# COPT-Public/LoRADS

Measured on AMD Instinct MI355X. Metric: ADMM iters/sec (+ inner CG-iters/sec), single-block n=20000 r=40, higher is better.
Workload: dtype f64

## Files before the change

include/lorads_hip.h:

```cpp
#ifndef LORADS_HIP_H
#define LORADS_HIP_H

#include <stdint.h>

#ifdef __cplusplus
extern "C" {
#endif

typedef struct lorads_hip_ctx lorads_hip_ctx;

typedef struct {
    int32_t n;
    int32_t rank;
    int32_t nrow;
    const int32_t *row_idx;
    const int32_t *a_ptr;
    const int32_t *a_row;
    const int32_t *a_col;
    const double *a_val;
    int32_t c_nnz;
    const int32_t *c_row;
    const int32_t *c_col;
    const double *c_val;
    int32_t is_lp;
// ... 70 lines not shown

int lorads_hip_primal_topk(lorads_hip_ctx *ctx, int32_t src, int32_t blk, int32_t nq, const int32_t *row, int32_t col_lo, int32_t col_hi,
                           int32_t k, int32_t smallest, int32_t include_diag, const int64_t *skip_ptr, const int32_t *skip_col,
                           int32_t *idx, double *val, int32_t *found);

int lorads_hip_alm_to_admm(lorads_hip_ctx *ctx);
int lorads_hip_average_uv_to_v(lorads_hip_ctx *ctx);
int lorads_hip_scale_obj(lorads_hip_ctx *ctx, double s);
int lorads_hip_resize_rank(lorads_hip_ctx *ctx, const int32_t *new_rank);
int lorads_hip_set_mat(lorads_hip_ctx *ctx, int32_t which, int32_t blk, const double *colmajor);
int lorads_hip_get_mat(lorads_hip_ctx *ctx, int32_t which, int32_t blk, double *colmajor);
int lorads_hip_set_vec(lorads_hip_ctx *ctx, int32_t which, const double *v);
int lorads_hip_get_vec(lorads_hip_ctx *ctx, int32_t which, double *v);
int lorads_hip_set_allreduce(lorads_hip_ctx *ctx, lorads_hip_allreduce_fn fn, void *user);
void *lorads_hip_stream(lorads_hip_ctx *ctx);
int lorads_hip_set_allreduce_stream_ordered(lorads_hip_ctx *ctx, int32_t on);
int lorads_hip_set_separable(lorads_hip_ctx *ctx, int32_t on);
typedef int (*lorads_hip_scalar_exchange_fn)(void *user, double *vals, int32_t n);
int lorads_hip_set_scalar_exchange(lorads_hip_ctx *ctx, lorads_hip_scalar_exchange_fn fn, void *user);
int lorads_hip_selfcheck_allreduce(lorads_hip_ctx *ctx);

int lorads_hip_sync(lorads_hip_ctx *ctx);
int lorads_hip_spec_front_stats(lorads_hip_ctx *ctx, int64_t out[4]);
int lorads_hip_row_deal_stats(lorads_hip_ctx *ctx, int32_t block, int out[3]);
int lorads_hip_wt_stores(lorads_hip_ctx *ctx, int *mask);

#ifdef __cplusplus
}
#endif
#endif
```

lorads_amd/csrc/hip/kernels.inc:

```
template <int LG, bool V2, int NS>
struct Slice {
    static constexpr int W = V2 ? 2 : 1;
    __device__ static __forceinline__ void load(const double *__restrict__ row, int r, int lane, double (&v)[NS][W]) {
#pragma unroll
        for (int c = 0; c < NS; ++c) {
            const int j = (lane + c * LG) * W;
            const bool ok = j < r;
            const int jc = ok ? j : 0;
            if (V2) {
                const double2 t = *(const double2 *)(row + jc);
                v[c][0] = ok ? t.x : 0.0;
                v[c][W - 1] = ok ? t.y : 0.0;
            } else {
                const double t = row[jc];
                v[c][0] = ok ? t : 0.0;
            }
        }
    }
};

enum { WT_R0 = 1, WT_RHS = 2, WT_CONTRIB = 4, WT_CG0 = 8, WT_AVG = 16, WT_OUT = 32, WT_ALL = 63,
       WT_DEFAULT = WT_R0 | WT_RHS | WT_CG0 | WT_AVG };
__device__ __forceinline__ void store16(double *p, size_t off, double a, double b, bool wt) {
    if (wt) {
// ... 827 lines not shown
    DS rho, rho_dual;
    int dual_on;
    int wmode;
    double *contrib;
    CGState *reset;
    int nreset;
    int wt;
};
__device__ __forceinline__ void front_cw_weights(const FrontCwArgs &A, double rho, double rho_dual, int i, double a, double &c1, double &c2) {
    const int g = A.row_idx ? A.row_idx[i] : i;
    const double cs0 = A.csum[g], bb = A.b[g], lam0 = A.lambda[g], cvv = A.cv[i], wu = A.w_uv[i];
    double m1;
    if (A.wmode == W_ADMM_V) {
        const double cs = cs0 + (wu - cvv);
        m1 = ((cs - bb) - wu) * rho - lam0;
    } else {
        double lam = lam0;
        if (A.dual_on) { const double l = lam0 + rho_dual * bb; lam = l + (-rho_dual) * cs0; }
        m1 = ((cs0 - bb) - cvv) * rho - lam;
    }
    c1 = a * m1;
    c2 = a * wu;
}
template <int NS, int EW, int KC = 0>
__global__ __launch_bounds__(TPB) void k_front_cw(int n, int rpw, FrontCwArgs A, const double *__restrict__ X, int r,
                                                  const double *__restrict__ xin, double *__restrict__ out,
                                                  double *__restrict__ rhs_out, double *__restrict__ part,
                                                  double *__restrict__ part_b, Guard g, Deferred d) {
    constexpr int LG = 8, W = 2, NH = EW / 8;
    using SL = Slice<LG, true, NS>;
    __shared__ double sh[8];
    extern __shared__ __attribute__((aligned(16))) double2 slotc[];
    if (A.reset && blockIdx.x == 0 && threadIdx.x < A.nreset) A.reset[threadIdx.x].done = 0;
    const Gate gt = gate_load(g);
    const double rho = dsv(A.rho), rho_dual = A.dual_on ? dsv(A.rho_dual) : 0.0;
    DefPriv dv{};
    if (d.st) dv = deferred_private(d);
    const int grp = threadIdx.x / LG, row = blockIdx.x * rpw + grp, lane = threadIdx.x % LG, l8 = lane & 7;
    const bool act = grp < rpw && row < n;
    const int rowc = act ? row : 0;
    const size_t base = (size_t)rowc * r;
    const int c0 = A.fc_ptr[rowc], c1e = act ? A.fc_ptr[rowc + 1] : c0;
    const int a0 = A.sl_ptr[rowc], a1r = A.sl_ptr[rowc + 1];
    const int a1 = act ? a1r : a0;
    const int cnt = a1 - a0;
    const size_t eb = (size_t)rowc * EW + l8;
    int qc[NH], kc[NH], dc[NH];
    double ac[NH];
#pragma unroll
    for (int h = 0; h < NH; ++h) { qc[h] = A.ell_col[eb + 8 * h]; kc[h] = A.ell_con[eb + 8 * h]; ac[h] = A.ell_a[eb + 8 * h]; dc[h] = A.ell_dst[eb + 8 * h]; }
    int tn = c0 + l8, tc = tn < c1e ? tn : (c1e > 0 ? c1e - 1 : 0);
    int qn = A.fc_col[tc];
    double svn = A.fc_val[tc];
    double xi[NS][W], rh[NS][W];
    SL::load(X + base, r, lane, xi);
    SL::load(xin + base, r, lane, rh);
    double k1[NH], k2[NH];
#pragma unroll
    for (int h = 0; h < NH; ++h) {
        front_cw_weights(A, rho, rho_dual, kc[h], ac[h], k1[h], k2[h]);
        const bool mine = l8 + 8 * h < cnt;
// ... 112 lines not shown
#pragma unroll
                    for (int c = 0; c < NS; ++c)
#pragma unroll
                        for (int w = 0; w < W; ++w) dsum += r0[c][w] * v[u][c][w];
                    dsum = group_sum<LG>(dsum);
                    mine = l8 == u0 + u ? dsum : mine;
                }
            }
            if (live && l8 + 8 * h < cnt2) store8(A.contrib, (size_t)dc[h], ac[h] * mine, A.wt & WT_CONTRIB);
        }
    }
    for (int t = a0 + EW; t < a1b; ++t) {
        double v[NS][W], dsum = 0.0;
        SL::load(X + (size_t)A.sl_col[t] * r, r, lane, v);
#pragma unroll
        for (int c = 0; c < NS; ++c)
#pragma unroll
            for (int w = 0; w < W; ++w) dsum += r0[c][w] * v[c][w];
        dsum = group_sum<LG>(dsum);
        if (live && l8 == 0) store8(A.contrib, (size_t)A.sl_dst[t], A.sl_a[t] * dsum, A.wt & WT_CONTRIB);
    }
    double two[2] = {act ? local : 0.0, act ? local_b : 0.0};
    block_sum_n<2>(two, sh);
    if (live && threadIdx.x == 0) { part[blockIdx.x] = two[0]; part_b[blockIdx.x] = two[1]; }
}

__global__ __launch_bounds__(TPB) void k_wsum(int nrow, int cw, const double *__restrict__ contrib, double *__restrict__ w_out, Guard g,
                                              InitArgs ia, int dual_on, DS rho_dual_s, int m_all,
                                              const double *__restrict__ b, const double *__restrict__ csum,
                                              double *__restrict__ lambda, double *__restrict__ part_ww = nullptr,
                                              CGState *reset = nullptr, int nreset = 0) {
    __shared__ double sh[8];
    if (reset && blockIdx.x == 0 && threadIdx.x < nreset) reset[threadIdx.x].done = 0;
    const Gate gt = gate_load(ia.st ? Guard{nullptr, g.need} : g);
    double iv[2] = {0.0, 0.0};
    if (ia.st) init_private(ia, iv);
    const int i = (blockIdx.x * TPB + threadIdx.x) / 8, lane = threadIdx.x & 7;
    const bool act = i < nrow;
    const int ic = act ? i : 0;
    const double *cp = contrib + (size_t)ic * cw;
    double s = 0.0;
    for (int t = lane; t < cw; t += 32) {
        double v[4];
#pragma unroll
        for (int u = 0; u < 4; ++u) v[u] = cp[t + 8 * u < cw ? t + 8 * u : lane];
#pragma unroll
        for (int u = 0; u < 4; ++u) s += t + 8 * u < cw ? v[u] : 0.0;
// ... 926 lines not shown
    double acc = 0.0;
    for (int col = threadIdx.x; col < ncols; col += TPB) {
        double w = cobj[col];
        for (int t = ptr[col]; t < ptr[col + 1]; ++t) w += -lambda[grow[t]] * a[t];
        acc += fabs(w < 0.0 ? w : 0.0);
    }
    acc = block_sum(acc, sh);
    if (threadIdx.x == 0) *out = acc;
}

__global__ __launch_bounds__(TPB) void k_publish(const unsigned long long *__restrict__ src, int nwords, unsigned long long *dst,
                                                 unsigned long long *flag, unsigned long long *seq_dev) {
    const unsigned long long seq = *seq_dev + 1;
    for (int i = threadIdx.x; i < nwords; i += TPB) dst[i] = src[i];
    __threadfence_system();
    __syncthreads();
    if (threadIdx.x == 0) {
        *seq_dev = seq;
        __atomic_store_n(flag, seq, __ATOMIC_RELEASE);
        __threadfence_system();
    }
}

struct EvalFinalArgs {
    const double *part_v, *part_d, *obj_part;
    int np, nobj;
    double *out;
    Guard g;
};
__global__ __launch_bounds__(TPB) void k_publish_final(EvalFinalArgs fa, const unsigned long long *src, int nwords,
                                                       unsigned long long *dst, unsigned long long *flag, unsigned long long *seq_dev) {
    __shared__ double sh[12];
    const unsigned long long seq = *seq_dev + 1;
    constexpr int PW = 4;
    unsigned long long pre[PW];
#pragma unroll
    for (int k = 0; k < PW; ++k) {
        const int i = threadIdx.x + k * TPB;
        pre[k] = __builtin_nontemporal_load(src + (i < nwords ? i : 0));
    }
    const bool live = !blocked(fa.g);
    const double *const pp[3] = {fa.part_v, fa.part_d, fa.obj_part ? fa.obj_part : fa.part_v};
    const int nn[3] = {fa.np, fa.np, fa.obj_part ? fa.nobj : 0};
    double t3[3];
    private_partials_n<3>(pp, nn, t3);
    block_sum_n<3>(t3, sh);
    const double v = t3[0], d = t3[1], o = t3[2];
    if (live && threadIdx.x == 0) { fa.out[0] = v; fa.out[1] = d; if (fa.obj_part) fa.out[2] = o; }
    const bool own = (const double *)src == fa.out;
#pragma unroll
    for (int k = 0; k < PW; ++k) {
        const int i = threadIdx.x + k * TPB;
        if (i >= nwords) continue;
        unsigned long long w = pre[k];
        if (live && own) {
            if (i == 0) w = (unsigned long long)__double_as_longlong(v);
            else if (i == 1) w = (unsigned long long)__double_as_longlong(d);
            else if (i == 2 && fa.obj_part) w = (unsigned long long)__double_as_longlong(o);
        }
        dst[i] = w;
    }
    if (!own || nwords > PW * TPB) {
        __threadfence();
        __syncthreads();
        for (int i = threadIdx.x; i < nwords; i += TPB) dst[i] = __builtin_nontemporal_load(src + i);
    }
    __threadfence_system();
    __syncthreads();
    if (threadIdx.x == 0) {
        *seq_dev = seq;
        __atomic_store_n(flag, seq, __ATOMIC_RELEASE);
        __threadfence_system();
    }
}
struct SepExtra;
__global__ __launch_bounds__(TPB) void k_publish_sep(const double *buf, double *scal, int with_obj, int nex, double *ex0, double *ex1,
                                                     double *ex2, double *ex3, const unsigned long long *src, int nwords,
                                                     unsigned long long *dst, unsigned long long *flag, unsigned long long *seq_dev) {
    const unsigned long long seq = *seq_dev + 1;
    if (threadIdx.x == 0) {
        scal[0] = buf[0];
        scal[1] = buf[1];
        if (with_obj) scal[2] = buf[2];
        scal[5] = buf[3];
        double *const ex[4] = {ex0, ex1, ex2, ex3};
        for (int k = 0; k < nex; ++k) *ex[k] = buf[4 + k];
    }
    __threadfence();
    __syncthreads();
    for (int i = threadIdx.x; i < nwords; i += TPB) dst[i] = __builtin_nontemporal_load(src + i);
    __threadfence_system();
    __syncthreads();
    if (threadIdx.x == 0) {
        *seq_dev = seq;
        __atomic_store_n(flag, seq, __ATOMIC_RELEASE);
        __threadfence_system();
// ... 616 lines not shown
```

lorads_amd/csrc/hip/lorads_hip.hip:

```cpp
#include <hip/hip_runtime.h>

#include <fcntl.h>
#include <sys/file.h>
#include <unistd.h>

#include <algorithm>
#include <chrono>
#include <cmath>
#include <cstdint>
#include <cstdio>
#include <cstring>
#include <map>
#include <string>
#include <atomic>
#include <mutex>
#include <thread>
#include <tuple>
#include <type_traits>
#include <utility>
#include <vector>

#include "lorads_hip.h"
#include "lorads_hip_dev.h"

// ... 607 lines not shown
    bool opt_dense_cache = true;
    bool opt_front_diag = true;
    bool opt_eval_diag = true;
    bool opt_fold_avg = true;
    bool opt_tile_update = true;
    bool avg_folded = false;
    bool opt_front_lds = true;
    bool opt_front_cw = true;
    bool opt_fuse_cg0 = true;
    int opt_row_deal = -1, row_deal_cus = 0;
    int opt_wt_stores = WT_DEFAULT;
    bool opt_spec_front = true;
    struct SpecFront {
        bool live = false;
        bool dual_seen = false;
        double rho = 0.0, rho_dual = 0.0;
        int wmode = 0;
        unsigned long long epoch = 0;
        CGState *reset = nullptr;
        int nreset = 0;
    } spec;
    unsigned long long spec_epoch = 0;
    long long n_spec_enq = 0, n_spec_adopt = 0, n_spec_discard = 0, n_spec_blocked = 0;
    bool opt_exact_refresh = false, opt_split_front = false;
    bool final_pending = false;
    EvalFinalArgs final_args;
    double *scal = nullptr;
    CGState *st = nullptr;
    CGState *st_shadow = nullptr;
    bool opt_lazy_scalars = true;
    bool opt_seg_carry_init = true;
    lorads_hip_scalar_exchange_fn sx = nullptr;
    void *sx_user = nullptr;
    bool sx_pending = false;
    int sx_with_obj = 0;
    long long n_sx = 0;
    bool opt_seg_virt = true;
    bool opt_seg_carry_dual = true;
    bool opt_seg_carry_restart = true;
    double *seg_rr_alt = nullptr;
    int *seg_tile_info = nullptr;
    bool opt_seg_carry = true;
    int *seg_tile_cone = nullptr;
    CGState *h_st = nullptr;
    double *h_scal = nullptr;
    std::vector<Ring> ring;
// ... 114 lines not shown
    c->opt_gram = env_on("LORADS_LBFGS_GRAM");
    c->opt_gram_single = getenv("LORADS_LBFGS_GRAM") && getenv("LORADS_LBFGS_GRAM")[0] == '2';
    c->opt_fuse_dir = env_on("LORADS_FUSE_DIR");
    c->opt_entry_bip = env_on("LORADS_ENTRY_BIP");
    c->opt_seg_carry = env_on("LORADS_SEG_CARRY");
    c->opt_seg_carry_init = env_on("LORADS_SEG_CARRY_INIT");
    c->opt_seg_virt = env_on("LORADS_SEG_VIRT");
    c->opt_seg_carry_dual = env_on("LORADS_SEG_CARRY_DUAL");
    c->opt_seg_carry_restart = env_on("LORADS_SEG_CARRY_RESTART");
    c->opt_cw_quad = env_on("LORADS_CW_QUAD");
    c->opt_front_cw = env_on("LORADS_FRONT_CW");
    c->opt_fuse_cg0 = env_on("LORADS_FUSE_CG0");
    c->opt_front_lds = env_on("LORADS_FRONT_LDS");
    {
        const char *v = getenv("LORADS_ROW_DEAL");
        c->opt_row_deal = (!v || !v[0] || v[0] == 'a') ? -1 : std::max(0, std::min(32, atoi(v)));
        int dev = 0;
        HC(hipGetDevice(&dev));
        HC(hipDeviceGetAttribute(&c->row_deal_cus, hipDeviceAttributeMultiprocessorCount, dev));
        if (getenv("LORADS_ROW_DEAL_CUS")) c->row_deal_cus = std::max(1, atoi(getenv("LORADS_ROW_DEAL_CUS")));
    }
    if (getenv("LORADS_WT_STORES") && getenv("LORADS_WT_STORES")[0]) c->opt_wt_stores = atoi(getenv("LORADS_WT_STORES")) & WT_ALL;
    c->opt_spec_front = env_on("LORADS_SPEC_FRONT");
    if (getenv("LORADS_SPEC_WINDOW")) c->spec_window = std::max(1, std::min(8, atoi(getenv("LORADS_SPEC_WINDOW"))));
    c->opt_fold_avg = env_on("LORADS_FOLD_AVG");
    c->opt_tile_update = env_on("LORADS_TILE_UPDATE");
    c->opt_eval_diag = env_on("LORADS_EVAL_DIAG");
    c->opt_front_diag = env_on("LORADS_FRONT_DIAG");
    c->opt_dense_cache = env_on("LORADS_DENSE_CACHE");
    c->opt_fuse_eval = env_on("LORADS_FUSE_EVAL");
    c->opt_dense_rem = env_on("LORADS_DENSE_REM");
    c->opt_exact_refresh = env_set("LORADS_EXACT_REFRESH");
    c->opt_split_front = env_set("LORADS_SPLIT_FRONT");
    c->scal = (double *)c->ctrl;
    c->st = (CGState *)(c->ctrl + 64 * sizeof(double));
    c->h_scal = (double *)c->h_ctrl;
    c->h_st = (CGState *)(c->h_ctrl + 64 * sizeof(double));
    HC(hipMemset(c->lambda, 0, sizeof(double) * (size_t)std::max(c->m, 1)));
    HC(hipMemset(c->csum, 0, sizeof(double) * (size_t)(c->m + 2)));
    HC(hipMemset(c->q12, 0, sizeof(double) * (size_t)(2 * c->m + 2)));
    HC(hipMemset(c->scal, 0, sizeof(double) * 64));
    HC(hipMemset(c->ring_ab, 0, sizeof(double) * (size_t)2 * c->L));
    HC(hipMemset(c->st, 0, sizeof(CGState) * (size_t)std::max(2 * c->nb, 1)));
    if (M.alloc(&c->st_shadow, (size_t)std::max(2 * c->nb, 1))) return 1;
    HC(hipMemset(c->st_shadow, 0, sizeof(CGState) * (size_t)std::max(2 * c->nb, 1)));
    c->persist = new PersistPlan();
// ... 862 lines not shown
    for (int i = 0; i < 16; ++i) ticks[i] = 0;
    if (c->persist && c->persist->valid && c->persist->stamps && c->persist_stamps) {
        HC(hipMemcpy(c->persist->h_stamps, c->persist->stamps, sizeof(unsigned long long) * 16, hipMemcpyDeviceToHost));
        for (int i = 0; i < 16; ++i) ticks[i] = c->persist->h_stamps[i];
        HC(hipMemset(c->persist->stamps, 0, sizeof(unsigned long long) * 16));
    }
    c->persist_stamps = enable != 0;
    return 0;
}

int lorads_hip_presolve_stats(lorads_hip_ctx *c, int64_t stats[2]) {
    spec_touch(c);
    stats[0] = c->n_dev_patterns;
    stats[1] = c->n_checked_patterns;
    return 0;
}

int lorads_hip_spec_front_stats(lorads_hip_ctx *c, int64_t out[4]) {
    if (!c || !out) return fail_msg("spec_front_stats: bad argument");
    out[0] = c->n_spec_enq; out[1] = c->n_spec_adopt; out[2] = c->n_spec_discard; out[3] = c->n_spec_blocked;
    return 0;
}

int lorads_hip_row_deal_stats(lorads_hip_ctx *c, int32_t k, int out[3]) {
    if (!c || !out) return fail_msg("row_deal_stats: bad argument");
    if (k < 0 || k >= c->nb) return fail_msg("bad block");
    const RowDeal rd = row_deal_of(c, c->blk[k]);
    out[0] = rd.rpw; out[1] = rd.grid; out[2] = c->row_deal_cus;
    return 0;
}

int lorads_hip_wt_stores(lorads_hip_ctx *c, int *mask) {
    if (!c || !mask) return fail_msg("wt_stores: bad argument");
    *mask = c->opt_wt_stores;
    return 0;
}

int lorads_hip_graph_stats(lorads_hip_ctx *c, int64_t stats[4]) {
    spec_touch(c);
    stats[0] = c->graphs ? c->graphs->n_capture : 0;
    stats[1] = c->graphs ? c->graphs->n_replay : 0;
    stats[2] = c->graphs ? (int64_t)c->graphs->map.size() : 0;
    stats[3] = graph_ok(c) ? 1 : 0;
    return 0;
}

// ... 24 lines not shown
```

lorads_amd/csrc/hip/sweep.inc:

```
#define LAUNCH_LDS(kern, grid, lds, ...)                                                             \
    do {                                                                                             \
        const int grid__ = (int)(grid);                                                              \
        if (c->pend.must_flush()) c->pend.flush(c);                                                  \
        if (grid__ > 0) { ++c->n_launch; hipLaunchKernelGGL(kern, dim3(grid__), dim3(TPB), (size_t)(lds), c->stream, __VA_ARGS__); } \
    } while (0)
#define LAUNCH(kern, grid, ...) LAUNCH_LDS(kern, grid, 0, __VA_ARGS__)
#include "pending.inc"

struct Shape {
    int lg, v2, ns;
};
inline Shape shape_for(int r) {
    Shape s;
    s.v2 = use_v2(r);
    s.lg = lg_for(r);
    const int w = s.v2 ? 2 : 1;
    s.ns = (r + s.lg * w - 1) / (s.lg * w);
    return s;
}
#define NS_SWITCH(LGV, V2V, ns, ...)                                     \
    switch (ns) {                                                        \
    case 1: { constexpr int LG_ = LGV; constexpr bool V2_ = V2V; constexpr int NS_ = 1; __VA_ARGS__; } break; \
    case 2: { constexpr int LG_ = LGV; constexpr bool V2_ = V2V; constexpr int NS_ = 2; __VA_ARGS__; } break; \
    case 3: { constexpr int LG_ = LGV; constexpr bool V2_ = V2V; constexpr int NS_ = 3; __VA_ARGS__; } break; \
// ... 377 lines not shown
};

struct Solve {
    Block *B;
    double *x;
    const double *V;
    CGState *st;
    Guard front;
    size_t len;
    int gv;
    int tile = 0, tile_w = 0;
};

FrontCwArgs front_cw_args(lorads_hip_ctx *c, const Block &B, double rho, int wmode) {
    FrontCwArgs A{};
    A.fc_ptr = B.fc_ptr; A.fc_col = B.fc_col; A.fc_val = B.fc_val; A.sl_ptr = B.cadj_ptr; A.sl_col = B.cadj_col; A.sl_con = B.cadj_con;
    A.sl_a = B.cadj_a; A.ell_col = B.cell_col; A.ell_con = B.cell_con; A.ell_a = B.cell_a; A.ell_dst = B.cell_dst; A.sl_dst = B.cadj_dst; A.csum = c->csum; A.b = c->b;
    A.lambda = c->lambda; A.cv = B.cv; A.w_uv = B.w_uv; A.row_idx = B.row_idx_identity ? nullptr : B.row_idx; A.rho = ds_rho(c, rho);
    A.wmode = wmode;
    A.contrib = B.w_contrib;
    A.wt = c->opt_wt_stores;
    return A;
}
int launch_front_cw(lorads_hip_ctx *c, const Solve &s, const FrontCwArgs &A, Guard g, Deferred d) {
    Block &B = *s.B;
    double *r = c->cr + B.off, *rhs = c->rhs + B.off;
    double *pA = part_slot(c, 18), *pB = part_slot(c, 1);
    const RowDeal rd = row_deal_of(c, B);
    const int grid = rd.grid;
    const int ns = (B.r + 15) / 16;
    const bool keep = c->pend.set_dual_used(false);
    FrontSample fs(c);
#define FCW(EWV) NS_SWITCH(8, true, ns, LAUNCH((k_front_cw<NS_, EWV>), grid, B.n, rd.rpw, A, s.V, B.r, (const double *)s.x, r, rhs, pA, pB, g, d))
#define FCWL(NSV, EWV) LAUNCH_LDS((k_front_cw<NSV, EWV, 4>), grid, sizeof(double2) * 32 * 4 * NSV * 8, B.n, rd.rpw, A, s.V, B.r, (const double *)s.x, r, rhs, pA, pB, g, d)
    if (c->opt_front_lds && ns <= 3) {
        if (B.cell_w == 8) { if (ns == 1) FCWL(1, 8); else if (ns == 2) FCWL(2, 8); else FCWL(3, 8); }
        else { if (ns == 1) FCWL(1, 16); else if (ns == 2) FCWL(2, 16); else FCWL(3, 16); }
    } else if (B.cell_w == 8) { FCW(8) } else { FCW(16) }
#undef FCWL
#undef FCW
    fs.done();
    c->pend.set_dual_used(keep);
    return grid;
}
void front_cw_started(lorads_hip_ctx *c, const Solve &s, int grid, double tol) {
    s.B->w0_ready = true;
    c->pend.post_init(c, s.st, part_slot(c, 18), grid, part_slot(c, 1), grid, tol, s.front);
}
bool front_carries_dual(const lorads_hip_ctx *c, const Solve &s, int wmode) {
    return c->pend.dual_rides(s.front) && wmode == W_ADMM && c->nb == 1;
}
bool spec_front_adopt(lorads_hip_ctx *c, const Solve &s, double rho, double tol, CGState *reset, int nreset);

void solve_front(lorads_hip_ctx *c, const Solve &s, double rho, double tol, CGState *reset = nullptr, int nreset = 0) {
    Block &B = *s.B;
    double *r = c->cr + B.off, *p = c->cp + B.off, *rhs = c->rhs + B.off;
    double *pA = part_slot(c, 18), *pB = part_slot(c, 1);
    WArgs wa{};
    wa.csum = c->csum; wa.b = c->b; wa.lambda = c->lambda; wa.cv = B.cv; wa.row_idx = B.row_idx_identity ? nullptr : B.row_idx; wa.rho = ds_rho(c, rho);
    B.w0_ready = false;
    if (front_cw_ok(c, B)) {
// ... 121 lines not shown
    } else {
        const Deferred d = c->pend.take_check_of(s.st);
        LAUNCH(k_cg_dir, s.gv, s.len, s.st, (int)DIR_BETA, r, p, g, d);
    }
}
void solve_iters(lorads_hip_ctx *c, const Solve &s, int k0, int k1, double tol, int maxit, bool fold_avg_last = false) {
    for (int k = k0; k < k1; ++k) {
        if (k > k0) solve_iter_tail(c, s, k - 1, tol, maxit);
        solve_iter_body(c, s, k, tol, maxit, fold_avg_last && k == k1 - 1);
    }
}
void refresh_after_solve(lorads_hip_ctx *c, Block &B, const int *need) {
    if (constr_by_recurrence(c, B) && B.t_uv_valid && B.nrow > 0) {
        const Deferred d = c->pend.take_check_behind(Guard{nullptr, need});
        LAUNCH(k_refresh_w, nblocks_for((size_t)B.nrow, TPB), B.nrow, (const double *)B.w_uv, B.cv, B.row_idx, c->csum,
               Guard{nullptr, need}, d, B.diag_only ? (const int *)B.diag_row : (const int *)nullptr,
               B.diag_only ? (const double *)B.diag_a : (const double *)nullptr);
        return;
    }
    constr_val(c, B, c->U + B.off, c->V + B.off, 1.0, B.cv, CV_DELTA, c->csum, Guard{nullptr, need});
}

void flush_final(lorads_hip_ctx *c);
int enqueue_publish(lorads_hip_ctx *c, size_t word0, size_t nwords) {
    if (c->sx_pending && (word0 > SX_WORD || word0 + nwords < SX_WORD + 4)) {
        const size_t w1 = std::max(word0 + nwords, (size_t)SX_WORD + 4);
        word0 = std::min(word0, (size_t)SX_WORD);
        nwords = w1 - word0;
    }
    int sep_with_obj = 0;
    SepExtra ex{};
    const bool sep = !c->final_pending && c->pend.take_sep(4, &sep_with_obj, &ex);
    c->pend.flush(c);
    ++c->pub_seq;
    if (sep) {
        LAUNCH(k_publish_sep, 1, (const double *)c->sepbuf, c->scal, sep_with_obj, ex.n, ex.p[0], ex.p[1], ex.p[2],
               ex.p[3], (const unsigned long long *)c->ctrl + word0, (int)nwords, (unsigned long long *)c->h_ctrl_dev + word0,
               c->h_flag_dev, c->seq_dev);
    } else if (c->final_pending) {
        LAUNCH(k_publish_final, 1, c->final_args, (const unsigned long long *)c->ctrl + word0, (int)nwords,
               (unsigned long long *)c->h_ctrl_dev + word0, c->h_flag_dev, c->seq_dev);
        c->final_pending = false;
    } else {
        LAUNCH(k_publish, 1, (const unsigned long long *)c->ctrl + word0, (int)nwords, (unsigned long long *)c->h_ctrl_dev + word0,
               c->h_flag_dev, c->seq_dev);
    }
    return 0;
}
int sx_exchange(lorads_hip_ctx *c) {
    if (!c->sx_pending) return 0;
    c->sx_pending = false;
    double v[4] = {c->h_scal[SX_WORD], c->h_scal[SX_WORD + 1], c->h_scal[SX_WORD + 2], c->h_scal[SX_WORD + 3]};
    if (!c->sx || c->sx(c->sx_user, v, 4)) return fail_msg("scalar exchange of separable shards failed (a rank that never arrived?)");
    c->n_sx++;
    c->h_scal[0] = v[0];
    c->h_scal[1] = v[1];
    if (c->sx_with_obj) c->h_scal[2] = v[2];
    c->h_scal[5] = v[3];
    return 0;
}
int wait_publish(lorads_hip_ctx *c) {
    const unsigned long long seq = c->pub_seq;
    if (c->launch_err) { const char *e = c->launch_err; c->launch_err = nullptr; hipStreamSynchronize(c->stream); return fail_msg(e); }
    {
        hipError_t le = hipGetLastError();
        if (le != hipSuccess) return fail("kernel launch", le);
    }
    volatile unsigned long long *f = c->h_flag;
    static const double limit_s = getenv("LORADS_HANDOVER_TIMEOUT_S") ? atof(getenv("LORADS_HANDOVER_TIMEOUT_S")) : 300.0;
// ... 33 lines not shown

Solve make_solve(lorads_hip_ctx *c, int k, int half, const int *need) {
    Block &B = c->blk[k];
    Solve s;
    s.B = &B;
    s.x = (half == 0 ? c->U : c->V) + B.off;
    s.V = (half == 0 ? c->V : c->U) + B.off;
    s.st = c->st + 2 * k + half;
    s.front = Guard{nullptr, need};
    s.len = (size_t)B.n * B.r;
    s.gv = std::min(grid1d(s.len), 512);
    if (B.diag_only && c->opt_tile_update) {
        const int rows = TPB / shape_for(B.r).lg, g = nblocks_for((size_t)B.n, rows);
        if (g <= c->maxpart && rows * B.r >= TPB / 2) { s.gv = g; s.tile = rows * B.r; s.tile_w = rows; }
    }
    return s;
}

bool spec_front_ok(lorads_hip_ctx *c) {
    if (!c->opt_spec_front || !c->use_publish || c->ar || c->nb != 1 || !c->opt_lazy_scalars || !c->lambda_alt) return false;
    if (c->prof && c->prof_every < (1 << 20)) return false;
    return front_cw_ok(c, c->blk[0]) && !c->blk[0].is_lp;
}
void spec_front_enqueue(lorads_hip_ctx *c, double rho) {
    Block &B = c->blk[0];
    if (!B.t_uv_valid || c->pend.dual_owed()) return;
    const Solve s = make_solve(c, 0, 0, nullptr);
    FrontCwArgs A = front_cw_args(c, B, rho, W_ADMM);
    A.dual_on = 1;
    A.rho_dual = ds_rho_dual(c, rho);
    launch_front_cw(c, s, A, Guard{nullptr, &c->st[2 * c->nb - 1].done}, Deferred{});
    c->spec.live = true; c->spec.dual_seen = false;
    c->spec.rho = rho; c->spec.rho_dual = rho; c->spec.wmode = W_ADMM; c->spec.epoch = c->spec_epoch;
    ++c->n_spec_enq;
}
bool spec_front_adopt(lorads_hip_ctx *c, const Solve &s, double rho, double tol, CGState *reset, int nreset) {
    if (!c->spec.live) return false;
    c->spec.live = false;
    Block &B = *s.B;
    const bool ok = s.st == c->st && reset && !c->par_mode && c->spec.epoch == c->spec_epoch && memcmp(&rho, &c->spec.rho, sizeof(double)) == 0 &&
                    c->spec.dual_seen && c->pend.dual_owed_at(c->spec.rho_dual) && !c->virt_refresh &&
                    c->spec.wmode == W_ADMM && front_carries_dual(c, s, W_ADMM) && B.t_uv_valid && c->opt_lazy_scalars &&
                    B.spec[0] >= 1;
    if (!ok) { ++c->n_spec_discard; return false; }
    ++c->n_spec_adopt;
    c->pend.use_dual();
    c->virt_refresh = false;
    c->spec.reset = reset; c->spec.nreset = nreset;
    c->n_front++;
    front_cw_started(c, s, row_deal_of(c, B).grid, tol);
    return true;
}

void enqueue_lp_sweep(lorads_hip_ctx *c, Block &B, double rho, CGState *st, Guard g) {
    c->pend.flush(c);
    LpArgs A;
    A.ncols = B.n; A.nlev = B.lp_nlev; A.lvl_ptr = B.lp_lvl_ptr; A.lvl_cols = B.lp_lvl_cols; A.ptr = B.lp_ptr; A.grow = B.lp_grow;
// ... 406 lines not shown
            const CGState &h = c->h_st[2 * k + half];
            if (h.done != 2) mx = std::max(mx, h.iter);
        }
        c->spec_b_hist[half][c->spec_b_pos % c->spec_window] = mx;
        int mw = 0;
        for (int k = 0; k < c->spec_window; ++k) mw = std::max(mw, c->spec_b_hist[half][k]);
        c->spec_b[half] = mw;
        if (half == 1) c->spec_b_pos++;
    }
    if (with_eval && c->ar && any_missed) {
        if (enqueue_eval(c, LORADS_HIP_PAIR_UV, nullptr)) return 1;
        if (read_states(c)) return 1;
    }
    return 0;
}

bool persist_ready(lorads_hip_ctx *c, int maxit);
int run_sweep_persist(lorads_hip_ctx *c, double rho, double tol, int maxit, bool with_eval);
int run_sweep(lorads_hip_ctx *c, double rho, double tol, int maxit, bool with_eval) {
    if (persist_ready(c, maxit)) { spec_touch(c); return run_sweep_persist(c, rho, tol, maxit, with_eval); }
    persist_touch(c);
    if (c->has_merged && !getenv("LORADS_NO_BATCH")) { spec_touch(c); return run_sweep_batched(c, rho, tol, maxit, with_eval); }
    int first = 0, resume = -1;
    bool first_pass = true, any_missed = false;
    const bool graph = graph_this_step(c, rho, tol, maxit);
    if (graph && set_step_params(c, rho, tol, maxit)) return 1;
    ParMode pm(c, graph);
    if (graph || maxit < 1) spec_touch(c);
    const bool spec = with_eval && !graph && spec_front_ok(c);
    for (;;) {
        const bool eval_now = with_eval && (!c->ar || first_pass);
        auto enq = [&]() -> int {
            if (first_pass && 2 * c->nb - 1 > TPB) HC(hipMemsetAsync(c->st, 0, sizeof(CGState) * (size_t)(2 * c->nb), c->stream));
            enqueue_sweep(c, first, resume, rho, tol, maxit, with_eval);
            if (eval_now && enqueue_eval(c, LORADS_HIP_PAIR_UV, c->nb ? &c->st[2 * c->nb - 1].done : nullptr)) return 1;
            return c->use_publish ? enqueue_publish(c, 0, state_words(c)) : 0;
        };
        if (graph && first_pass) {
            std::vector<uint64_t> key{1, (uint64_t)with_eval, (uint64_t)maxit, (uint64_t)((c->n_sweeps % 32) == 31)};
            if (graph_step(c, key, enq)) return 1;
        } else if (enq()) return 1;
        if (spec && first_pass) spec_front_enqueue(c, rho);
        if (c->use_publish ? wait_publish(c) : read_states(c)) return 1;
        if (eval_now && c->ar) any_missed = c->h_scal[5] > 0.5;
        const int stg = first_unfinished(c, first);
        if (first_pass && c->spec.live && stg >= 0) { c->spec.live = false; ++c->n_spec_blocked; }
        first_pass = false;
        if (stg < 0) break;
        first = stg;
        resume = c->h_st[stg].iter;
        c->n_resume++;
        c->merged.t_uv_valid = false;
        for (auto &B : c->blk) { B.t_uv_valid = false; B.w0_ready = false; B.wj_for = nullptr; }
    }
    if (with_eval && c->ar && any_missed) {
        if (enqueue_eval(c, LORADS_HIP_PAIR_UV, nullptr)) return 1;
        if (read_states(c)) return 1;
    }
    c->n_sweeps++;
    return 0;
}
```

lorads_amd/host.py:

```python
import ctypes as C
import os

import numpy as np

_HERE = os.path.dirname(os.path.abspath(__file__))
LIB_DIR = os.path.join(_HERE, "lib")
DEV_LIB = os.path.join(LIB_DIR, "liblorads_hip_dev.so")

PAIR_RR, PAIR_UV = 0, 1
MAT_R, MAT_U, MAT_V, MAT_GRAD = 0, 1, 2, 3
VEC_LAMBDA, VEC_CONSTR_SUM, VEC_Q1, VEC_Q2 = 0, 1, 2, 3

_dp = C.POINTER(C.c_double)
_ip = C.POINTER(C.c_int)
ALLREDUCE_FN = C.CFUNCTYPE(C.c_int, C.c_void_p, C.c_void_p, C.c_int, C.c_int)


class BackendStruct(C.Structure):
    _fields_ = [
        ("ctx", C.c_void_p),
        ("name", C.c_char_p),
        ("init_constr", C.CFUNCTYPE(C.c_int, C.c_void_p, C.c_int)),
        ("alm_cal_grad", C.CFUNCTYPE(C.c_int, C.c_void_p, C.c_double, _dp)),
        ("lbfgs_direction", C.CFUNCTYPE(C.c_int, C.c_void_p, C.c_int)),
# ... 579 lines not shown
        nnz = C.c_int64()
        _check(lib.lorads_hip_get_slack(ctx, int(blk), C.byref(nnz), None, None, None), "get_slack")
        row, col, val = np.zeros(nnz.value, dtype=np.int32), np.zeros(nnz.value, dtype=np.int32), np.zeros(nnz.value)
        _check(lib.lorads_hip_get_slack(ctx, int(blk), C.byref(nnz), row.ctypes.data_as(i32p), col.ctypes.data_as(i32p),
                                        val.ctypes.data_as(_dp)), "get_slack")
        return row, col, val

    def hip_block_image(self, blk=0):
        lib, ctx = self._hip()
        out = (C.c_int64 * 16)()
        lib.lorads_hip_block_image.argtypes = [C.c_void_p, C.c_int, C.POINTER(C.c_int64)]
        _check(lib.lorads_hip_block_image(ctx, blk, out), "block_image")
        keys = ["n", "rank", "nrow", "na", "nc", "pattern_a", "pattern_union", "dense_c", "dense_a", "diag_only", "entry_only", "use_cw",
                "has_gram", "front_cw", "slot_width", "bip_rows0"]
        return dict(zip(keys, [int(out[i]) for i in range(16)]))

    def hip_spec_front_stats(self):
        lib, ctx = self._hip()
        out = (C.c_int64 * 4)()
        lib.lorads_hip_spec_front_stats.argtypes = [C.c_void_p, C.POINTER(C.c_int64)]
        _check(lib.lorads_hip_spec_front_stats(ctx, out), "spec_front_stats")
        return dict(zip(["enqueued", "adopted", "discarded", "blocked"], [int(out[i]) for i in range(4)]))

    def hip_row_deal_stats(self, blk=0):
        lib, ctx = self._hip()
        out = (C.c_int * 3)()
        lib.lorads_hip_row_deal_stats.argtypes = [C.c_void_p, C.c_int32, C.POINTER(C.c_int)]
        _check(lib.lorads_hip_row_deal_stats(ctx, blk, out), "row_deal_stats")
        return dict(zip(["rpw", "grid", "ncu"], [int(out[i]) for i in range(3)]))

    def hip_wt_stores(self):
        lib, ctx = self._hip()
        out = C.c_int(-1)
        lib.lorads_hip_wt_stores.argtypes = [C.c_void_p, C.POINTER(C.c_int)]
        _check(lib.lorads_hip_wt_stores(ctx, C.byref(out)), "wt_stores")
        return int(out.value)

    def hip_graph_stats(self):
        lib, ctx = self._hip()
        out = (C.c_int64 * 4)()
        lib.lorads_hip_graph_stats.argtypes = [C.c_void_p, C.POINTER(C.c_int64)]
        _check(lib.lorads_hip_graph_stats(ctx, out), "graph_stats")
        return dict(zip(["captured", "replayed", "held", "enabled"], [int(out[i]) for i in range(4)]))

    def hip_persist_stats(self):
        lib, ctx = self._hip()
# ... 500 lines not shown
```

profiles/trace_summary.py:

```python
#!/usr/bin/env python3
import collections
import csv
import re
import statistics
import sys

rows = list(csv.DictReader(open(sys.argv[1])))
rows.sort(key=lambda r: int(r["Start_Timestamp"]))


PHASE1_MARKS = ("k_his_two", "k_lbfgs_team", "k_alm_close")


def short(n):
    m = re.search(r"(k_\w+|__amd_\w+)", n)
    return m.group(1) if m else n[:40]


last = max(i for i, r in enumerate(rows) if any(k in r["Kernel_Name"] for k in PHASE1_MARKS))
alm = len(sys.argv) > 2 and sys.argv[2] == "alm"
adm = rows[:last + 1] if alm else rows[last + 1:]
if alm:
    print("inner iterations (k_his_two / k_lbfgs_team launches): %d" % sum(1 for r in adm if "k_his_two" in r["Kernel_Name"] or "k_lbfgs_team" in r["Kernel_Name"]))
t0 = int(adm[0]["Start_Timestamp"])
t1 = int(adm[-1]["End_Timestamp"])
print(("ALM-part" if alm else "ADMM-part") + " kernels: %d  span %.3f ms" % (len(adm), (t1 - t0) / 1e6))
agg = collections.OrderedDict()
for r in adm:
    k = short(r["Kernel_Name"])
    d = int(r["End_Timestamp"]) - int(r["Start_Timestamp"])
    a = agg.setdefault(k, [0, 0, []])
    a[0] += 1
    a[1] += d
    a[2].append(d)
tot = sum(v[1] for v in agg.values())
for k, v in sorted(agg.items(), key=lambda x: -x[1][1]):
    print("%-30s calls %5d  total %9.1f us  avg %7.2f us  med %7.2f us  %5.1f%%" %
          (k, v[0], v[1] / 1e3, v[1] / v[0] / 1e3, statistics.median(v[2]) / 1e3, 100 * v[1] / tot))
print("sum of kernel time %.3f ms, busy fraction %.2f" % (tot / 1e6, tot / (t1 - t0)))
gaps = [int(adm[i + 1]["Start_Timestamp"]) - int(adm[i]["End_Timestamp"]) for i in range(len(adm) - 1)]
print("gaps: median %.2f us  mean %.2f us  max %.1f us  (>20us: %d)" %
      (statistics.median(gaps) / 1e3, sum(gaps) / len(gaps) / 1e3, max(gaps) / 1e3, sum(1 for g in gaps if g > 20000)))
```

Baseline: 9628.

## Fold final publish into speculative front kernel as an extra workgroup

Moves the publish_final body into a device function. When a speculative front kernel is about to be enqueued, workgroup 0 of k_front_cw now runs the final reduction and host handover, and the remaining workgroups run the front rows with an offset index. This removes a separate single-block k_publish_final launch and its launch gap from each ADMM step. The cost is one extra workgroup in the front grid and a new template variant, and the path depends on env flags and on the spec-front conditions holding.

After: 10040 (median of 6 runs). 1.04x the previous value.

```diff
diff --git a/include/lorads_hip.h b/include/lorads_hip.h
--- a/include/lorads_hip.h
+++ b/include/lorads_hip.h
@@ -116,6 +116,7 @@
 
 int lorads_hip_sync(lorads_hip_ctx *ctx);
 int lorads_hip_spec_front_stats(lorads_hip_ctx *ctx, int64_t out[4]);
+int lorads_hip_handover_stats(lorads_hip_ctx *ctx, int64_t out[2]);
 int lorads_hip_row_deal_stats(lorads_hip_ctx *ctx, int32_t block, int out[3]);
 int lorads_hip_wt_stores(lorads_hip_ctx *ctx, int *mask);
 
diff --git a/lorads_amd/csrc/hip/kernels.inc b/lorads_amd/csrc/hip/kernels.inc
--- a/lorads_amd/csrc/hip/kernels.inc
+++ b/lorads_amd/csrc/hip/kernels.inc
@@ -873,21 +873,88 @@
     c1 = a * m1;
     c2 = a * wu;
 }
-template <int NS, int EW, int KC = 0>
-__global__ __launch_bounds__(TPB) void k_front_cw(int n, int rpw, FrontCwArgs A, const double *__restrict__ X, int r,
+struct EvalFinalArgs {
+    const double *part_v, *part_d, *obj_part;
+    int np, nobj;
+    double *out;
+    Guard g;
+};
+__device__ __forceinline__ void publish_final(EvalFinalArgs fa, const unsigned long long *src, int nwords, unsigned long long *dst,
+                                              unsigned long long *flag, unsigned long long *seq_dev, double *sh) {
+    const unsigned long long seq = *seq_dev + 1;
+    constexpr int PW = 4;
+    unsigned long long pre[PW];
+#pragma unroll
+    for (int k = 0; k < PW; ++k) {
+        const int i = threadIdx.x + k * TPB;
+        pre[k] = __builtin_nontemporal_load(src + (i < nwords ? i : 0));
+    }
+    const bool live = !blocked(fa.g);
+    const double *const pp[3] = {fa.part_v, fa.part_d, fa.obj_part ? fa.obj_part : fa.part_v};
+    const int nn[3] = {fa.np, fa.np, fa.obj_part ? fa.nobj : 0};
+    double t3[3];
+    private_partials_n<3>(pp, nn, t3);
+    block_sum_n<3>(t3, sh);
+    const double v = t3[0], d = t3[1], o = t3[2];
+    if (live && threadIdx.x == 0) { fa.out[0] = v; fa.out[1] = d; if (fa.obj_part) fa.out[2] = o; }
+    const bool own = (const double *)src == fa.out;
+#pragma unroll
+    for (int k = 0; k < PW; ++k) {
+        const int i = threadIdx.x + k * TPB;
+        if (i >= nwords) continue;
+        unsigned long long w = pre[k];
+        if (live && own) {
+            if (i == 0) w = (unsigned long long)__double_as_longlong(v);
+            else if (i == 1) w = (unsigned long long)__double_as_longlong(d);
+            else if (i == 2 && fa.obj_part) w = (unsigned long long)__double_as_longlong(o);
+        }
+        dst[i] = w;
+    }
+    if (!own || nwords > PW * TPB) {
+        __threadfence();
+        __syncthreads();
+        for (int i = threadIdx.x; i < nwords; i += TPB) dst[i] = __builtin_nontemporal_load(src + i);
+    }
+    __threadfence_system();
+    __syncthreads();
+    if (threadIdx.x == 0) {
+        *seq_dev = seq;
+        __atomic_store_n(flag, seq, __ATOMIC_RELEASE);
+        __threadfence_system();
+    }
+}
+struct HandoverArgs {
+    EvalFinalArgs fa;
+    const unsigned long long *src;
+    unsigned long long *dst;
+    int nwords;
+    unsigned long long *flag, *seq_dev;
+};
+struct FrontCwHoArgs : FrontCwArgs { HandoverArgs ho; };
+template <int NS, int EW, int KC = 0, bool HO = false>
+__global__ __launch_bounds__(TPB) void k_front_cw(int n, int rpw, std::conditional_t<HO, FrontCwHoArgs, FrontCwArgs> A,
+                                                  const double *__restrict__ X, int r,
                                                   const double *__restrict__ xin, double *__restrict__ out,
                                                   double *__restrict__ rhs_out, double *__restrict__ part,
                                                   double *__restrict__ part_b, Guard g, Deferred d) {
     constexpr int LG = 8, W = 2, NH = EW / 8;
     using SL = Slice<LG, true, NS>;
-    __shared__ double sh[8];
+    __shared__ double sh[HO ? 12 : 8];
     extern __shared__ __attribute__((aligned(16))) double2 slotc[];
-    if (A.reset && blockIdx.x == 0 && threadIdx.x < A.nreset) A.reset[threadIdx.x].done = 0;
+    unsigned wg = blockIdx.x;
+    if constexpr (HO) {
+        if (blockIdx.x == 0) {
+            publish_final(A.ho.fa, A.ho.src, A.ho.nwords, A.ho.dst, A.ho.flag, A.ho.seq_dev, sh);
+            return;
+        }
+        wg = blockIdx.x - 1;
+    }
+    if (A.reset && wg == 0 && threadIdx.x < A.nreset) A.reset[threadIdx.x].done = 0;
     const Gate gt = gate_load(g);
     const double rho = dsv(A.rho), rho_dual = A.dual_on ? dsv(A.rho_dual) : 0.0;
     DefPriv dv{};
     if (d.st) dv = deferred_private(d);
-    const int grp = threadIdx.x / LG, row = blockIdx.x * rpw + grp, lane = threadIdx.x % LG, l8 = lane & 7;
+    const int grp = threadIdx.x / LG, row = wg * rpw + grp, lane = threadIdx.x % LG, l8 = lane & 7;
     const bool act = grp < rpw && row < n;
     const int rowc = act ? row : 0;
     const size_t base = (size_t)rowc * r;
@@ -1046,7 +1113,7 @@
     }
     double two[2] = {act ? local : 0.0, act ? local_b : 0.0};
     block_sum_n<2>(two, sh);
-    if (live && threadIdx.x == 0) { part[blockIdx.x] = two[0]; part_b[blockIdx.x] = two[1]; }
+    if (live && threadIdx.x == 0) { part[wg] = two[0]; part_b[wg] = two[1]; }
 }
 
 __global__ __launch_bounds__(TPB) void k_wsum(int nrow, int cw, const double *__restrict__ contrib, double *__restrict__ w_out, Guard g,
@@ -2019,56 +2086,10 @@
     }
 }
 
-struct EvalFinalArgs {
-    const double *part_v, *part_d, *obj_part;
-    int np, nobj;
-    double *out;
-    Guard g;
-};
 __global__ __launch_bounds__(TPB) void k_publish_final(EvalFinalArgs fa, const unsigned long long *src, int nwords,
                                                        unsigned long long *dst, unsigned long long *flag, unsigned long long *seq_dev) {
     __shared__ double sh[12];
-    const unsigned long long seq = *seq_dev + 1;
-    constexpr int PW = 4;
-    unsigned long long pre[PW];
-#pragma unroll
-    for (int k = 0; k < PW; ++k) {
-        const int i = threadIdx.x + k * TPB;
-        pre[k] = __builtin_nontemporal_load(src + (i < nwords ? i : 0));
-    }
-    const bool live = !blocked(fa.g);
-    const double *const pp[3] = {fa.part_v, fa.part_d, fa.obj_part ? fa.obj_part : fa.part_v};
-    const int nn[3] = {fa.np, fa.np, fa.obj_part ? fa.nobj : 0};
-    double t3[3];
-    private_partials_n<3>(pp, nn, t3);
-    block_sum_n<3>(t3, sh);
-    const double v = t3[0], d = t3[1], o = t3[2];
-    if (live && threadIdx.x == 0) { fa.out[0] = v; fa.out[1] = d; if (fa.obj_part) fa.out[2] = o; }
-    const bool own = (const double *)src == fa.out;
-#pragma unroll
-    for (int k = 0; k < PW; ++k) {
-        const int i = threadIdx.x + k * TPB;
-        if (i >= nwords) continue;
-        unsigned long long w = pre[k];
-        if (live && own) {
-            if (i == 0) w = (unsigned long long)__double_as_longlong(v);
-            else if (i == 1) w = (unsigned long long)__double_as_longlong(d);
-            else if (i == 2 && fa.obj_part) w = (unsigned long long)__double_as_longlong(o);
-        }
-        dst[i] = w;
-    }
-    if (!own || nwords > PW * TPB) {
-        __threadfence();
-        __syncthreads();
-        for (int i = threadIdx.x; i < nwords; i += TPB) dst[i] = __builtin_nontemporal_load(src + i);
-    }
-    __threadfence_system();
-    __syncthreads();
-    if (threadIdx.x == 0) {
-        *seq_dev = seq;
-        __atomic_store_n(flag, seq, __ATOMIC_RELEASE);
-        __threadfence_system();
-    }
+    publish_final(fa, src, nwords, dst, flag, seq_dev, sh);
 }
 struct SepExtra;
 __global__ __launch_bounds__(TPB) void k_publish_sep(const double *buf, double *scal, int with_obj, int nex, double *ex0, double *ex1,
diff --git a/lorads_amd/csrc/hip/lorads_hip.hip b/lorads_amd/csrc/hip/lorads_hip.hip
--- a/lorads_amd/csrc/hip/lorads_hip.hip
+++ b/lorads_amd/csrc/hip/lorads_hip.hip
@@ -653,6 +653,8 @@
     } spec;
     unsigned long long spec_epoch = 0;
     long long n_spec_enq = 0, n_spec_adopt = 0, n_spec_discard = 0, n_spec_blocked = 0;
+    bool opt_handover_on_front = true;
+    long long n_handover_front = 0, n_handover_alone = 0;
     bool opt_exact_refresh = false, opt_split_front = false;
     bool final_pending = false;
     EvalFinalArgs final_args;
@@ -813,6 +815,7 @@
     }
     if (getenv("LORADS_WT_STORES") && getenv("LORADS_WT_STORES")[0]) c->opt_wt_stores = atoi(getenv("LORADS_WT_STORES")) & WT_ALL;
     c->opt_spec_front = env_on("LORADS_SPEC_FRONT");
+    c->opt_handover_on_front = env_on("LORADS_HANDOVER_ON_FRONT");
     if (getenv("LORADS_SPEC_WINDOW")) c->spec_window = std::max(1, std::min(8, atoi(getenv("LORADS_SPEC_WINDOW"))));
     c->opt_fold_avg = env_on("LORADS_FOLD_AVG");
     c->opt_tile_update = env_on("LORADS_TILE_UPDATE");
@@ -1721,6 +1724,12 @@
     return 0;
 }
 
+int lorads_hip_handover_stats(lorads_hip_ctx *c, int64_t out[2]) {
+    if (!c || !out) return fail_msg("handover_stats: bad argument");
+    out[0] = c->n_handover_front; out[1] = c->n_handover_alone;
+    return 0;
+}
+
 int lorads_hip_row_deal_stats(lorads_hip_ctx *c, int32_t k, int out[3]) {
     if (!c || !out) return fail_msg("row_deal_stats: bad argument");
     if (k < 0 || k >= c->nb) return fail_msg("bad block");
diff --git a/lorads_amd/csrc/hip/sweep.inc b/lorads_amd/csrc/hip/sweep.inc
--- a/lorads_amd/csrc/hip/sweep.inc
+++ b/lorads_amd/csrc/hip/sweep.inc
@@ -423,7 +423,7 @@
     A.wt = c->opt_wt_stores;
     return A;
 }
-int launch_front_cw(lorads_hip_ctx *c, const Solve &s, const FrontCwArgs &A, Guard g, Deferred d) {
+int launch_front_cw(lorads_hip_ctx *c, const Solve &s, const FrontCwArgs &A, Guard g, Deferred d, const HandoverArgs *ho = nullptr) {
     Block &B = *s.B;
     double *r = c->cr + B.off, *rhs = c->rhs + B.off;
     double *pA = part_slot(c, 18), *pB = part_slot(c, 1);
@@ -432,12 +432,17 @@
     const int ns = (B.r + 15) / 16;
     const bool keep = c->pend.set_dual_used(false);
     FrontSample fs(c);
-#define FCW(EWV) NS_SWITCH(8, true, ns, LAUNCH((k_front_cw<NS_, EWV>), grid, B.n, rd.rpw, A, s.V, B.r, (const double *)s.x, r, rhs, pA, pB, g, d))
-#define FCWL(NSV, EWV) LAUNCH_LDS((k_front_cw<NSV, EWV, 4>), grid, sizeof(double2) * 32 * 4 * NSV * 8, B.n, rd.rpw, A, s.V, B.r, (const double *)s.x, r, rhs, pA, pB, g, d)
-    if (c->opt_front_lds && ns <= 3) {
-        if (B.cell_w == 8) { if (ns == 1) FCWL(1, 8); else if (ns == 2) FCWL(2, 8); else FCWL(3, 8); }
-        else { if (ns == 1) FCWL(1, 16); else if (ns == 2) FCWL(2, 16); else FCWL(3, 16); }
-    } else if (B.cell_w == 8) { FCW(8) } else { FCW(16) }
+    FrontCwHoArgs AH{};
+    if (ho) { static_cast<FrontCwArgs &>(AH) = A; AH.ho = *ho; }
+#define FCW(EWV, HO, AV) NS_SWITCH(8, true, ns, LAUNCH((k_front_cw<NS_, EWV, 0, HO>), grid + HO, B.n, rd.rpw, AV, s.V, B.r, (const double *)s.x, r, rhs, pA, pB, g, d))
+#define FCWL(NSV, EWV, HO, AV) LAUNCH_LDS((k_front_cw<NSV, EWV, 4, HO>), grid + HO, sizeof(double2) * 32 * 4 * NSV * 8, B.n, rd.rpw, AV, s.V, B.r, (const double *)s.x, r, rhs, pA, pB, g, d)
+#define FRONT(HO, AV)                                                                                                    \
+    if (c->opt_front_lds && ns <= 3) {                                                                                   \
+        if (B.cell_w == 8) { if (ns == 1) FCWL(1, 8, HO, AV); else if (ns == 2) FCWL(2, 8, HO, AV); else FCWL(3, 8, HO, AV); }     \
+        else { if (ns == 1) FCWL(1, 16, HO, AV); else if (ns == 2) FCWL(2, 16, HO, AV); else FCWL(3, 16, HO, AV); }                \
+    } else if (B.cell_w == 8) { FCW(8, HO, AV) } else { FCW(16, HO, AV) }
+    if (ho) { FRONT(true, AH) } else { FRONT(false, A) }
+#undef FRONT
 #undef FCWL
 #undef FCW
     fs.done();
@@ -605,7 +610,8 @@
 }
 
 void flush_final(lorads_hip_ctx *c);
-int enqueue_publish(lorads_hip_ctx *c, size_t word0, size_t nwords) {
+bool spec_front_enqueue(lorads_hip_ctx *c, double rho, const HandoverArgs *ho = nullptr);
+int enqueue_publish(lorads_hip_ctx *c, size_t word0, size_t nwords, const double *front_rho = nullptr, bool *front_carried = nullptr) {
     if (c->sx_pending && (word0 > SX_WORD || word0 + nwords < SX_WORD + 4)) {
         const size_t w1 = std::max(word0 + nwords, (size_t)SX_WORD + 4);
         word0 = std::min(word0, (size_t)SX_WORD);
@@ -621,13 +627,22 @@
                ex.p[3], (const unsigned long long *)c->ctrl + word0, (int)nwords, (unsigned long long *)c->h_ctrl_dev + word0,
                c->h_flag_dev, c->seq_dev);
     } else if (c->final_pending) {
-        LAUNCH(k_publish_final, 1, c->final_args, (const unsigned long long *)c->ctrl + word0, (int)nwords,
-               (unsigned long long *)c->h_ctrl_dev + word0, c->h_flag_dev, c->seq_dev);
+        const HandoverArgs H{c->final_args, (const unsigned long long *)c->ctrl + word0, (unsigned long long *)c->h_ctrl_dev + word0,
+                             (int)nwords, c->h_flag_dev, c->seq_dev};
+        const bool own = (const double *)H.src == H.fa.out;
+        if (front_rho && c->opt_handover_on_front && own && spec_front_enqueue(c, *front_rho, &H)) {
+            *front_carried = true;
+            c->final_pending = false;
+            ++c->n_handover_front;
+            return 0;
+        }
+        LAUNCH(k_publish_final, 1, H.fa, H.src, H.nwords, H.dst, H.flag, H.seq_dev);
         c->final_pending = false;
     } else {
         LAUNCH(k_publish, 1, (const unsigned long long *)c->ctrl + word0, (int)nwords, (unsigned long long *)c->h_ctrl_dev + word0,
                c->h_flag_dev, c->seq_dev);
     }
+    ++c->n_handover_alone;
     return 0;
 }
 int sx_exchange(lorads_hip_ctx *c) {
@@ -707,17 +722,18 @@
     if (c->prof && c->prof_every < (1 << 20)) return false;
     return front_cw_ok(c, c->blk[0]) && !c->blk[0].is_lp;
 }
-void spec_front_enqueue(lorads_hip_ctx *c, double rho) {
+bool spec_front_enqueue(lorads_hip_ctx *c, double rho, const HandoverArgs *ho) {
     Block &B = c->blk[0];
-    if (!B.t_uv_valid || c->pend.dual_owed()) return;
+    if (!B.t_uv_valid || c->pend.dual_owed()) return false;
     const Solve s = make_solve(c, 0, 0, nullptr);
     FrontCwArgs A = front_cw_args(c, B, rho, W_ADMM);
     A.dual_on = 1;
     A.rho_dual = ds_rho_dual(c, rho);
-    launch_front_cw(c, s, A, Guard{nullptr, &c->st[2 * c->nb - 1].done}, Deferred{});
+    launch_front_cw(c, s, A, Guard{nullptr, &c->st[2 * c->nb - 1].done}, Deferred{}, ho);
     c->spec.live = true; c->spec.dual_seen = false;
     c->spec.rho = rho; c->spec.rho_dual = rho; c->spec.wmode = W_ADMM; c->spec.epoch = c->spec_epoch;
     ++c->n_spec_enq;
+    return true;
 }
 bool spec_front_adopt(lorads_hip_ctx *c, const Solve &s, double rho, double tol, CGState *reset, int nreset) {
     if (!c->spec.live) return false;
@@ -1170,7 +1186,7 @@
     persist_touch(c);
     if (c->has_merged && !getenv("LORADS_NO_BATCH")) { spec_touch(c); return run_sweep_batched(c, rho, tol, maxit, with_eval); }
     int first = 0, resume = -1;
-    bool first_pass = true, any_missed = false;
+    bool first_pass = true, any_missed = false, front_carried = false;
     const bool graph = graph_this_step(c, rho, tol, maxit);
     if (graph && set_step_params(c, rho, tol, maxit)) return 1;
     ParMode pm(c, graph);
@@ -1182,13 +1198,14 @@
             if (first_pass && 2 * c->nb - 1 > TPB) HC(hipMemsetAsync(c->st, 0, sizeof(CGState) * (size_t)(2 * c->nb), c->stream));
             enqueue_sweep(c, first, resume, rho, tol, maxit, with_eval);
             if (eval_now && enqueue_eval(c, LORADS_HIP_PAIR_UV, c->nb ? &c->st[2 * c->nb - 1].done : nullptr)) return 1;
-            return c->use_publish ? enqueue_publish(c, 0, state_words(c)) : 0;
+            if (!c->use_publish) return 0;
+            return enqueue_publish(c, 0, state_words(c), spec && first_pass ? &rho : nullptr, &front_carried);
         };
         if (graph && first_pass) {
             std::vector<uint64_t> key{1, (uint64_t)with_eval, (uint64_t)maxit, (uint64_t)((c->n_sweeps % 32) == 31)};
             if (graph_step(c, key, enq)) return 1;
         } else if (enq()) return 1;
-        if (spec && first_pass) spec_front_enqueue(c, rho);
+        if (spec && first_pass && !front_carried) spec_front_enqueue(c, rho);
         if (c->use_publish ? wait_publish(c) : read_states(c)) return 1;
         if (eval_now && c->ar) any_missed = c->h_scal[5] > 0.5;
         const int stg = first_unfinished(c, first);
diff --git a/lorads_amd/host.py b/lorads_amd/host.py
--- a/lorads_amd/host.py
+++ b/lorads_amd/host.py
@@ -625,6 +625,13 @@
         _check(lib.lorads_hip_spec_front_stats(ctx, out), "spec_front_stats")
         return dict(zip(["enqueued", "adopted", "discarded", "blocked"], [int(out[i]) for i in range(4)]))
 
+    def hip_handover_stats(self):
+        lib, ctx = self._hip()
+        out = (C.c_int64 * 2)()
+        lib.lorads_hip_handover_stats.argtypes = [C.c_void_p, C.POINTER(C.c_int64)]
+        _check(lib.lorads_hip_handover_stats(ctx, out), "handover_stats")
+        return dict(zip(["on_front", "alone"], [int(out[i]) for i in range(2)]))
+
     def hip_row_deal_stats(self, blk=0):
         lib, ctx = self._hip()
         out = (C.c_int * 3)()
diff --git a/profiles/trace_summary.py b/profiles/trace_summary.py
--- a/profiles/trace_summary.py
+++ b/profiles/trace_summary.py
@@ -38,6 +38,12 @@
     print("%-30s calls %5d  total %9.1f us  avg %7.2f us  med %7.2f us  %5.1f%%" %
           (k, v[0], v[1] / 1e3, v[1] / v[0] / 1e3, statistics.median(v[2]) / 1e3, 100 * v[1] / tot))
 print("sum of kernel time %.3f ms, busy fraction %.2f" % (tot / 1e6, tot / (t1 - t0)))
+by_pred = collections.OrderedDict()
+for prev, r in zip(adm, adm[1:]):
+    if short(r["Kernel_Name"]) == "k_front_cw":
+        by_pred.setdefault(short(prev["Kernel_Name"]), []).append(int(r["End_Timestamp"]) - int(r["Start_Timestamp"]))
+for k, v in by_pred.items():
+    print("k_front_cw behind %-22s calls %5d  med %7.2f us" % (k, len(v), statistics.median(v) / 1e3))
 gaps = [int(adm[i + 1]["Start_Timestamp"]) - int(adm[i]["End_Timestamp"]) for i in range(len(adm) - 1)]
 print("gaps: median %.2f us  mean %.2f us  max %.1f us  (>20us: %d)" %
       (statistics.median(gaps) / 1e3, sum(gaps) / len(gaps) / 1e3, max(gaps) / 1e3, sum(1 for g in gaps if g > 20000)))
```
